# lin-shuyu/ladder-latent-data-distribution-modelling

Hardware: AMD Instinct MI355X
Metric: training images/sec (full 4-run LaDDer iteration, CelebA 128x128) (higher is better)
Workload: dtype f32; 1 GPU; BASELINE configs[2]: celeba 128x128x3 nh=512 z=64 R=2 K=30 L=100 per-GPU batch=128, 4 runs/iteration (AE step, sigma step, prior step, inner-sigma step), fitted-GM regime; global_batch=128, parallelism=dp1

## Files before the change

### include/ladder_hip.h

```cpp
#ifndef LADDER_HIP_H
#define LADDER_HIP_H

#include <stddef.h>
#include <stdint.h>

#ifdef __cplusplus
extern "C" {
#endif

typedef struct ihipStream_t* ladder_stream_t;

enum { LADDER_OK = 0, LADDER_E_SHAPE = -1, LADDER_E_ALIGN = -2, LADDER_E_WORKSPACE = -3, LADDER_E_LAUNCH = -4 };
enum { LADDER_ACT_NONE = 0, LADDER_ACT_LEAKY = 1 , LADDER_ACT_RELU = 2, LADDER_ACT_TANH = 3 };

#define LADDER_ABI_VERSION 2
int ladder_abi_version(void);
int ladder_igemm_fwd_tile(long M, int Cin, int Cout);
int ladder_conv2d_fwd_kernel_id(int N, int H, int W, int Cin, int Ho, int Wo, int Cout, int KH, int KW, int stride, int ups,
                                int pad_t, int pad_l);
int ladder_dense_fwd_nt(const float* x, const float* wT, const float* bias, float* y, int M, int K, int N, int act, ladder_stream_t stream);
int ladder_dense_bwd_data_nt(const float* dy, const float* w, float* dx, int M, int K, int N, const float* gate_y, int gate_act, ladder_stream_t stream);
int ladder_dense_fwd_is_persistent(long M, int K, int N);
int ladder_dense_bwd_weight_is_persistent(long M, int K, int N);

// ... 187 lines not shown

int ladder_conv_rgb_s2_eligible(int N, int H, int W, int Cin, int Cout, int KH, int KW, int stride, int pad_t, int pad_l);
int ladder_conv_rgb_s2_fwd(const float* x, const float* w, const float* bias, float* y, int N, int H, int W, int Cout, int act,
                           ladder_stream_t stream);
size_t ladder_conv_rgb_s2_fwd_bnstats_workspace_bytes(int N, int H, int W, int Cout);
int ladder_conv_rgb_s2_fwd_bnstats(const float* x, const float* w, const float* bias, float* y, int N, int H, int W, int Cout, int act,
                                   float* sums4 , void* ws, size_t ws_bytes,
                                   ladder_stream_t stream);
int ladder_conv_rgb_s2_fwd_f32(const float* x, const float* w, const float* bias, float* y, int N, int H, int W, int Cout, int act,
                               ladder_stream_t stream);
int ladder_conv_rgb_s2_fwd_bnstats_f32(const float* x, const float* w, const float* bias, float* y, int N, int H, int W, int Cout, int act,
                                       float* sums, void* ws, size_t ws_bytes, ladder_stream_t stream);
int ladder_conv_rgb_s2_bwd_filter_f32(const float* x, const float* dy, float* dw, float* db, int N, int H, int W, int Cout, void* ws,
                                      size_t ws_bytes, ladder_stream_t stream);
size_t ladder_conv_rgb_s2_bwd_filter_workspace_bytes(int N, int H, int W, int Cout);
int ladder_conv_rgb_s2_bwd_filter(const float* x, const float* x_absmax, const float* dy, const float* dy_absmax, float* dw, float* db,
                                  int N, int H, int W, int Cout, void* ws, size_t ws_bytes, ladder_stream_t stream);

int ladder_act_bwd(const float* dy, const float* y, float* dx, size_t n, int act, ladder_stream_t stream);

size_t ladder_bn_workspace_bytes(size_t rows, int C);
int ladder_bn_fwd_stats(const float* x, float* sums , size_t rows, int C,
                        void* ws, size_t ws_bytes, ladder_stream_t stream);
int ladder_bn_stats_from_partials(const float* partials, int nblk, float* sums , int C, ladder_stream_t stream);
int ladder_bn_fwd_stats_minmax(const float* x, float* sums4, size_t rows, int C, void* ws, size_t ws_bytes, ladder_stream_t stream);
int ladder_bn_stats_minmax_from_partials(const float* partials , int nblk, float* sums4, int C, ladder_stream_t stream);
int ladder_bn_fwd_apply_planes(const float* x, const float* sums4, double count, const float* gamma, const float* beta, float* y,
                               void* y_planes, float* mean_rstd, size_t rows, int C, float eps, int act, float* y_absmax,
                               ladder_stream_t stream);
int ladder_bn_fwd_apply(const float* x, const float* sums, double count,
                        const float* gamma, const float* beta, float* y, float* mean_rstd,
                        size_t rows, int C, float eps, int act, ladder_stream_t stream);
int ladder_bn_bwd_stats(const float* dy, const float* x, const float* mean_rstd, const float* gamma,
                        const float* beta, float* dsums , size_t rows, int C, int act,
                        void* ws, size_t ws_bytes, ladder_stream_t stream);
int ladder_bn_bwd_apply(const float* dy, const float* x, const float* mean_rstd, const float* gamma,
                        const float* beta, const float* dsums, double count, float* dx,
                        float* dgamma, float* dbeta, size_t rows, int C, int act, ladder_stream_t stream);
int ladder_bn_fwd_apply_absmax(const float* x, const float* sums, double count, const float* gamma, const float* beta, float* y,
// ... 245 lines not shown
```

### ladder_latent_data_distribution_modelling_amd/_lib.py

```python
import ctypes as C
import os

_HERE = os.path.dirname(os.path.abspath(__file__))
LIB_PATH = os.path.join(_HERE, "csrc", "libladder_hip.so")

ERRORS = {-1: "LADDER_E_SHAPE", -2: "LADDER_E_ALIGN", -3: "LADDER_E_WORKSPACE", -4: "LADDER_E_LAUNCH"}
ACT = {None: 0, "none": 0, "leaky_relu": 1, "relu": 2, "tanh": 3}

P_PIX_ABS, P_PIX_SQ, P_LOG_SDZ, P_MU2SD2_Z, P_CODE_ERR, P_CODE_SQRT, P_CODE_ABS, P_LOG_SDT, P_MU2SD2_T, P_LOGP = range(10)
P_FIXED = 16
S_NAMES = ["sigma", "mean_pixel_error", "entropy_z", "crossEntropy_prior_sg", "crossEntropy_prior",
           "l1_reconstruction_error", "l2_reconstruction_error", "reconstruction_likelihood", "sigma_regularisor",
           "elbo", "loss_ae", "inner_sigma", "mean_code_error", "code_reconstruction_likelihood",
           "code_l1_reconstruction_error", "representation_regularisor", "entropy_t",
           "crossEntropy_representation", "elbo_prior", "loss_prior",
           "_g_pix", "_g_sigma_var", "_g_code", "_g_inner_sigma_var", "_inv_B", "_inv_LB"]
S_INDEX = {n: i for i, n in enumerate(S_NAMES)}
S_COUNT = 32
ABSMAX_FLOATS = 512
ABI_VERSION = 2


class LadderElboCfg(C.Structure):
    _fields_ = [("B_global", C.c_int), ("D", C.c_int), ("Z", C.c_int), ("R", C.c_int), ("L", C.c_int),
# ... 186 lines not shown
    "ladder_dense_bwd_small": (_i, [_p, _p, _p, _p, _p, _p, _i, _i, _i, _p, _i, _p]),
    "ladder_dense_fwd_small_f32": (_i, [_p, _p, _p, _p, _i, _i, _i, _i, _p]),
    "ladder_dense_bwd_data_small_f32": (_i, [_p, _p, _p, _i, _i, _i, _p, _i, _p]),
    "ladder_dense_bwd_weight_small_f32": (_i, [_p, _p, _p, _p, _i, _i, _i, _p]),
    "ladder_dense_bwd_small_f32": (_i, [_p, _p, _p, _p, _p, _p, _i, _i, _i, _p, _i, _p]),
    "ladder_presplit_bytes": (_z, [_z, _i]),
    "ladder_presplit": (_i, [_p, _p, _p, _z, _i, _i, _p]),
    "ladder_absmax_samples": (_i, [_p, _i, _z, _p, _p]),
    "ladder_conv3x3_split_proj": (_i, [_p, _p, _p, _p, _p, _p, _p, _p] + [_i] * 8 + [_p]),
    "ladder_conv_rgb_s2_eligible": (_i, [_i] * 10),
    "ladder_conv_rgb_s2_fwd": (_i, [_p, _p, _p, _p, _i, _i, _i, _i, _i, _p]),
    "ladder_conv_rgb_s2_fwd_bnstats_workspace_bytes": (_z, [_i] * 4),
    "ladder_conv_rgb_s2_fwd_bnstats": (_i, [_p, _p, _p, _p, _i, _i, _i, _i, _i, _p, _p, _z, _p]),
    "ladder_conv_rgb_s2_fwd_f32": (_i, [_p, _p, _p, _p, _i, _i, _i, _i, _i, _p]),
    "ladder_conv_rgb_s2_fwd_bnstats_f32": (_i, [_p, _p, _p, _p, _i, _i, _i, _i, _i, _p, _p, _z, _p]),
    "ladder_bn_stats_from_partials": (_i, [_p, _i, _p, _i, _p]),
    "ladder_bn_stats_minmax_from_partials": (_i, [_p, _i, _p, _i, _p]),
    "ladder_bn_fwd_stats_minmax": (_i, [_p, _p, _z, _i, _p, _z, _p]),
    "ladder_bn_fwd_apply_planes": (_i, [_p, _p, _d, _p, _p, _p, _p, _p, _z, _i, _f, _i, _p, _p]),
    "ladder_conv_rgb_s2_bwd_filter_workspace_bytes": (_z, [_i] * 4),
    "ladder_conv_rgb_s2_bwd_filter": (_i, [_p] * 6 + [_i] * 4 + [_p, _z, _p]),
    "ladder_conv_rgb_s2_bwd_filter_f32": (_i, [_p] * 4 + [_i] * 4 + [_p, _z, _p]),
    "ladder_bn_fwd_apply_absmax": (_i, [_p, _p, _d, _p, _p, _p, _p, _z, _i, _f, _i, _p, _p]),
    "ladder_bn_bwd_apply_absmax": (_i, [_p, _p, _p, _p, _p, _p, _d, _p, _p, _p, _z, _i, _i, _p, _p]),
    "ladder_in_style_fwd_absmax": (_i, [_p, _p, _p, _p, _i, _i, _i, _f, _i, _p, _z, _p, _p]),
    "ladder_in_style_fwd_resize2x": (_i, [_p, _p, _p, _p, _i, _i, _i, _i, _f, _i, _p, _z, _p, _p]),
    "ladder_in_style_fwd_resize2x_keep": (_i, [_p, _p, _p, _p, _p, _i, _i, _i, _i, _f, _i, _p, _z, _p, _p]),
    "ladder_in_style_bwd_absmax": (_i, [_p, _p, _p, _p, _p, _p, _i, _i, _i, _i, _p, _z, _p, _p]),
    "ladder_conv1x1_smallcout_bwd_absmax": (_i, [_p, _p, _p, _p, _p, _p, C.c_long, _i, _i, _i, _p, _z, _p, C.c_long, _p]),
    "ladder_absmax": (_i, [_p, _z, _p, _p]),
    "ladder_conv3x3_wgrad_split_eligible": (_i, [_i] * 6),
# ... 78 lines not shown
```

### ladder_latent_data_distribution_modelling_amd/csrc/convrgb.hip

```cpp
#include "split16.h"
#include "igemm.h"

namespace {

constexpr int RGB_TH = 8, RGB_TW = 32, RGB_PIX = RGB_TH * RGB_TW;
constexpr int RGB_PH = 2 * RGB_TH + 1, RGB_PW = 2 * RGB_TW + 1;
constexpr int RGB_PATCH = RGB_PH * RGB_PW * 3;
constexpr int RGB_THREADS = 512;
constexpr int RGB_A_PLANE = 2 * 2 * RGB_PIX * 16;
constexpr int RGB_B_PLANE = 2 * 2 * 128 * 16;

__device__ __forceinline__ float block_max_512(float m, float* red) {
  m = wave_max(m);
  __syncthreads();
  if ((threadIdx.x & 63) == 0) red[threadIdx.x >> 6] = m;
  __syncthreads();
  float b = red[0];
#pragma unroll
  for (int w = 1; w < 8; ++w) b = fmaxf(b, red[w]);
  return b;
}

__device__ __forceinline__ float rgb_tap(const float* __restrict__ patch, int pr, int pc, int k) {
  const int tap = k / 3, ci = k - tap * 3, r = tap / 3, s = tap - r * 3;
  return patch[((2 * pr + r) * RGB_PW + 2 * pc + s) * 3 + ci];
}

constexpr int RGB_K32 = 28, RGB_LDA32 = RGB_K32 + 1;
template <bool F32>
__global__ __launch_bounds__(RGB_THREADS, 4) void conv_rgb_s2_fwd_kernel(const float* __restrict__ x, const float* __restrict__ w,
                                                                        const float* __restrict__ bias, float* __restrict__ y,
                                                                        const int N, const int H, const int W, const int Cout,
                                                                        const int act, const int tiles_n, float* __restrict__ stats_part) {
  __shared__ __attribute__((aligned(16))) unsigned char lds[2 * RGB_A_PLANE + 2 * RGB_B_PLANE];
  __shared__ __attribute__((aligned(16))) float patch[RGB_PATCH + 5];
  __shared__ float red[8];
  unsigned char* const Ab = lds;
  unsigned char* const Bb = lds + 2 * RGB_A_PLANE;

  const int tid = threadIdx.x, lane = tid & 63, wid = tid >> 6;
  const int l31 = lane & 31, lh = lane >> 5, wm = wid >> 1, wn = wid & 1;
  const int Ho = H / 2, Wo = W / 2;
  const int tile = blockIdx.x, mt = tile / tiles_n, cot = tile - mt * tiles_n, n0 = cot * 128;
  const int tw_n = Wo / RGB_TW, th_n = Ho / RGB_TH;
  const int img = mt / (tw_n * th_n), rem = mt - img * (tw_n * th_n);
  const int h0 = (rem / tw_n) * RGB_TH, w0 = (rem % tw_n) * RGB_TW;

  float xmax = 0.f;
// ... 107 lines not shown
#pragma unroll
        for (int mi = 0; mi < 2; ++mi)
#pragma unroll
          for (int ni = 0; ni < 2; ++ni) acc[mi][ni] = mfma16<true>(a[mi][pa], b[ni][sum - pa], acc[mi][ni]);
  }

  }

  const float unscale = 1.f / (cx * cw);
  float st0[2] = {0.f, 0.f}, st1[2] = {0.f, 0.f};
  float smn[2] = {INFINITY, INFINITY}, smx[2] = {-INFINITY, -INFINITY};
#pragma unroll
  for (int ni = 0; ni < 2; ++ni) {
    const int n = n0 + wn * 64 + ni * 32 + l31;
    const float bv = (bias != nullptr && n < Cout) ? bias[n] : 0.f;
#pragma unroll
    for (int mi = 0; mi < 2; ++mi) {
      float* yp = y + (((long)img * Ho + h0 + 2 * wm + mi) * Wo + w0) * Cout + n;
#pragma unroll
      for (int e = 0; e < 16; ++e) {
        const int px = (e & 3) + 8 * (e >> 2) + 4 * lh;
        const float v = ladder_act_fn(acc[mi][ni][e] * unscale + bv, act);
        if (n < Cout) yp[(long)px * Cout] = v;
        st0[ni] += v;
        st1[ni] += v * v;
        smn[ni] = fminf(smn[ni], v);
        smx[ni] = fmaxf(smx[ni], v);
      }
    }
  }
  if (stats_part != nullptr) {
    float* sred = reinterpret_cast<float*>(lds);
    __syncthreads();
#pragma unroll
    for (int ni = 0; ni < 2; ++ni) {
      const float a0 = st0[ni] + __shfl_xor(st0[ni], 32, 64), a1 = st1[ni] + __shfl_xor(st1[ni], 32, 64);
      const float a2 = fminf(smn[ni], __shfl_xor(smn[ni], 32, 64)), a3 = fmaxf(smx[ni], __shfl_xor(smx[ni], 32, 64));
      if (lh == 0) {
// ... 221 lines not shown
    __syncthreads();
  }

  float* o = part + (size_t)split * 27 * Cout;
#pragma unroll
  for (int e = 0; e < 16; ++e) {
    const int k = (e & 3) + 8 * (e >> 2) + 4 * lh;
    if (k < 27 && co_ok) o[(size_t)k * Cout + co] = acc[e];
  }
  if (bias_part != nullptr) {
    const float v = bsum + __shfl_down(bsum, 32, 64);
    if (lh == 0 && co_ok) bias_part[(size_t)split * Cout + co] = v;
  }
}

struct RgbWgradPlan { int tiles_co, splits, pps; };
RgbWgradPlan plan_rgb_wgrad(int N, int H, int W, int Cout) {
  RgbWgradPlan p;
  p.tiles_co = (Cout + 127) / 128;
  const long q_total = (long)N * (H / 2 / RW_PH) * (W / 2 / RW_PW);
  long s = (3 * 256L) / p.tiles_co;
  if (s > q_total / 4) s = q_total / 4;
  if (s < 1) s = 1;
  p.pps = (int)((q_total + s - 1) / s);
  p.splits = (int)((q_total + p.pps - 1) / p.pps);
  return p;
}

bool rgb_s2_ok(int N, int H, int W, int Cin, int Cout, int KH, int KW, int stride, int pad_t, int pad_l) {
  return N > 0 && Cin == 3 && KH == 3 && KW == 3 && stride == 2 && pad_t == 0 && pad_l == 0 && (H % 2) == 0 && (W % 2) == 0 &&
         ((H / 2) % RGB_TH) == 0 && ((W / 2) % RGB_TW) == 0 && Cout >= 32 && (Cout % 4) == 0;
}

}

extern "C" {

int ladder_conv_rgb_s2_eligible(int N, int H, int W, int Cin, int Cout, int KH, int KW, int stride, int pad_t, int pad_l) {
  return rgb_s2_ok(N, H, W, Cin, Cout, KH, KW, stride, pad_t, pad_l) ? 1 : 0;
}

static int rgb_fwd_launch(const float* x, const float* w, const float* bias, float* y, int N, int H, int W, int Cout, int act, float* stats_part,
                          ladder_stream_t stream, bool f32 = false) {
  if (!rgb_s2_ok(N, H, W, 3, Cout, 3, 3, 2, 0, 0)) return LADDER_E_SHAPE;
  if (!ladder_aligned16(y) || (bias != nullptr && !ladder_aligned16(bias))) return LADDER_E_ALIGN;
  const int tiles_n = (Cout + 127) / 128;
  const long tiles = (long)N * (H / 2 / RGB_TH) * (W / 2 / RGB_TW) * tiles_n;
  if (tiles >= (1L << 31)) return LADDER_E_SHAPE;
  if (f32)
    hipLaunchKernelGGL(conv_rgb_s2_fwd_kernel<true>, dim3((unsigned)tiles), dim3(RGB_THREADS), 0, stream, x, w, bias, y, N, H, W, Cout, act, tiles_n,
                       stats_part);
  else
    hipLaunchKernelGGL(conv_rgb_s2_fwd_kernel<false>, dim3((unsigned)tiles), dim3(RGB_THREADS), 0, stream, x, w, bias, y, N, H, W, Cout, act, tiles_n,
                       stats_part);
  LADDER_CHECK_LAUNCH();
  return LADDER_OK;
}

int ladder_conv_rgb_s2_fwd(const float* x, const float* w, const float* bias, float* y, int N, int H, int W, int Cout, int act,
                           ladder_stream_t stream) {
  return rgb_fwd_launch(x, w, bias, y, N, H, W, Cout, act, nullptr, stream);
}

size_t ladder_conv_rgb_s2_fwd_bnstats_workspace_bytes(int N, int H, int W, int Cout) {
  if (!rgb_s2_ok(N, H, W, 3, Cout, 3, 3, 2, 0, 0)) return 0;
  return (size_t)N * (H / 2 / RGB_TH) * (W / 2 / RGB_TW) * 4 * Cout * sizeof(float);
}

int ladder_conv_rgb_s2_fwd_bnstats(const float* x, const float* w, const float* bias, float* y, int N, int H, int W, int Cout, int act,
// ... 4 lines not shown
  const int rc = rgb_fwd_launch(x, w, bias, y, N, H, W, Cout, act, (float*)ws, stream);
  if (rc != LADDER_OK) return rc;
  return ladder_bn_stats_minmax_from_partials((const float*)ws, N * (H / 2 / RGB_TH) * (W / 2 / RGB_TW), sums, Cout, stream);
}

int ladder_conv_rgb_s2_fwd_f32(const float* x, const float* w, const float* bias, float* y, int N, int H, int W, int Cout, int act,
                               ladder_stream_t stream) {
  return rgb_fwd_launch(x, w, bias, y, N, H, W, Cout, act, nullptr, stream, true);
}

int ladder_conv_rgb_s2_fwd_bnstats_f32(const float* x, const float* w, const float* bias, float* y, int N, int H, int W, int Cout, int act,
                                       float* sums, void* ws, size_t ws_bytes, ladder_stream_t stream) {
  const size_t need = ladder_conv_rgb_s2_fwd_bnstats_workspace_bytes(N, H, W, Cout);
  if (need == 0 || sums == nullptr) return LADDER_E_SHAPE;
  if (ws == nullptr || ws_bytes < need) return LADDER_E_WORKSPACE;
  const int rc = rgb_fwd_launch(x, w, bias, y, N, H, W, Cout, act, (float*)ws, stream, true);
  if (rc != LADDER_OK) return rc;
  return ladder_bn_stats_minmax_from_partials((const float*)ws, N * (H / 2 / RGB_TH) * (W / 2 / RGB_TW), sums, Cout, stream);
}

int ladder_conv_rgb_s2_bwd_filter_f32(const float* x, const float* dy, float* dw, float* db, int N, int H, int W, int Cout, void* ws,
                                      size_t ws_bytes, ladder_stream_t stream) {
  if (!rgb_s2_ok(N, H, W, 3, Cout, 3, 3, 2, 0, 0)) return LADDER_E_SHAPE;
  if (!ladder_aligned16(dw)) return LADDER_E_ALIGN;
  const RgbWgradPlan p = plan_rgb_wgrad(N, H, W, Cout);
  if (ws == nullptr || ws_bytes < (size_t)p.splits * (27 * (size_t)Cout + Cout) * sizeof(float)) return LADDER_E_WORKSPACE;
  const WgradTail t = wgrad_tail(ws, p.splits, (size_t)27 * Cout, Cout, dw, db);
  hipLaunchKernelGGL(conv_rgb_s2_wgrad_f32_kernel, dim3(p.tiles_co * p.splits), dim3(RW_THREADS), 0, stream, x, dy, t.part, t.bias_part, N, H, W, Cout,
                     p.tiles_co, p.pps);
  return t.reduce(stream);
}

size_t ladder_conv_rgb_s2_bwd_filter_workspace_bytes(int N, int H, int W, int Cout) {
  if (!rgb_s2_ok(N, H, W, 3, Cout, 3, 3, 2, 0, 0)) return 0;
  const RgbWgradPlan p = plan_rgb_wgrad(N, H, W, Cout);
  return (size_t)p.splits * (27 * (size_t)Cout + Cout) * sizeof(float);
}

int ladder_conv_rgb_s2_bwd_filter(const float* x, const float* x_absmax, const float* dy, const float* dy_absmax, float* dw, float* db, int N,
                                  int H, int W, int Cout, void* ws, size_t ws_bytes, ladder_stream_t stream) {
  if (!rgb_s2_ok(N, H, W, 3, Cout, 3, 3, 2, 0, 0) || x_absmax == nullptr || dy_absmax == nullptr) return LADDER_E_SHAPE;
  if (!ladder_aligned16(dy) || !ladder_aligned16(dw)) return LADDER_E_ALIGN;
  if (ws == nullptr || ws_bytes < ladder_conv_rgb_s2_bwd_filter_workspace_bytes(N, H, W, Cout)) return LADDER_E_WORKSPACE;
  const RgbWgradPlan p = plan_rgb_wgrad(N, H, W, Cout);
  const WgradTail t = wgrad_tail(ws, p.splits, (size_t)27 * Cout, Cout, dw, db);
  hipLaunchKernelGGL(conv_rgb_s2_wgrad_kernel, dim3(p.tiles_co * p.splits), dim3(RW_THREADS), 0, stream, x, dy, t.part, t.bias_part, N, H, W, Cout,
                     p.tiles_co, p.pps, x_absmax, dy_absmax);
// ... 5 lines not shown
```

### ladder_latent_data_distribution_modelling_amd/csrc/norm.hip

```cpp
#include "split16.h"
#include "norm_util.h"

namespace {

template <bool MINMAX>
struct MomentsRow {
  using Sum = double;
  static constexpr bool kMinMax = MINMAX;
  const float* x;
  double* ws;
  float* wsmm;
  template <int V> struct Coef {};
  template <int V> using In = Lanes<float, V>;
  template <int V> struct Acc {
    Lanes<double, V> s0 = lanes_fill<double, V>(0.0), s1 = lanes_fill<double, V>(0.0);
    Lanes<float, V> mn = lanes_fill<float, V>(INFINITY), mx = lanes_fill<float, V>(-INFINITY);
  };
  template <int V> __device__ __forceinline__ Coef<V> coef(int, int) const { return {}; }
  template <int V> __device__ __forceinline__ In<V> load(size_t i) const { return lanes_load<V>(x + i); }
  template <int V> __device__ __forceinline__ void add(Acc<V>& a, const In<V>& v, const Coef<V>&) const {
#pragma unroll
    for (int j = 0; j < V; ++j) {
      const double d = (double)v.v[j];
      a.s0.v[j] += d;
// ... 863 lines not shown

int ladder_bn_bwd_stats(const float* dy, const float* x, const float* mean_rstd, const float* gamma, const float* beta,
                        float* dsums, size_t rows, int C, int act, void* ws, size_t ws_bytes, ladder_stream_t stream) {
  if (rows == 0 || C <= 0) return LADDER_E_SHAPE;
  const size_t nblk = stats_nblk(rows);
  if (ws_bytes < nblk * 2 * (size_t)C * sizeof(float)) return LADDER_E_WORKSPACE;
  const BnBwdRow row = {dy, x, mean_rstd, gamma, beta, (float*)ws, act};
  if (vec4_ok(C, x, dy)) stage1_launch<4>(row, rows, C, nblk, stream);
  else stage1_launch<1>(row, rows, C, nblk, stream);
  hipLaunchKernelGGL((colstats_stage2<64, 16, 1, false, float, float>), dim3((2 * C + 63) / 64), dim3(1024), 0, stream, (const float*)ws, 2,
                     (const float*)nullptr, 0, 0, dsums, (int)nblk, C);
  LADDER_CHECK_LAUNCH();
  return LADDER_OK;
}

int ladder_bn_bwd_apply(const float* dy, const float* x, const float* mean_rstd, const float* gamma, const float* beta,
                        const float* dsums, double count, float* dx, float* dgamma, float* dbeta, size_t rows, int C, int act,
                        ladder_stream_t stream) {
  return ladder_bn_bwd_apply_absmax(dy, x, mean_rstd, gamma, beta, dsums, count, dx, dgamma, dbeta, rows, C, act, nullptr, stream);
}

int ladder_bn_bwd_apply_absmax(const float* dy, const float* x, const float* mean_rstd, const float* gamma, const float* beta,
                               const float* dsums, double count, float* dx, float* dgamma, float* dbeta, size_t rows, int C, int act,
                               float* dx_absmax, ladder_stream_t stream) {
  if (rows == 0 || C <= 0 || count <= 0) return LADDER_E_SHAPE;
  const size_t n = rows * (size_t)C;
  const bool v4 = dx != nullptr && vec4_ok(C, x, dy, dx);
  if (dx_absmax != nullptr && !v4) return LADDER_E_SHAPE;
  const bool pgrad = dgamma != nullptr && dbeta != nullptr;
  static const bool fold = getenv("LADDER_DISABLE_BN_FOLD") == nullptr;
// ... 191 lines not shown
```

### ladder_latent_data_distribution_modelling_amd/engine.py

```python
import os

import numpy as np
import torch

from . import _lib as L
from . import arch
from . import layers as _layers
from .comm import Comm, VirtualComm, VirtualGroup, run_virtual_ranks, _NoComm, _DoneWork, _TracedWork
from .layers import (ADAM_B1, ADAM_B2, ADAM_EPS, BN_EPS, DEFAULT_PRECISION, IN_EPS, PRECISION_NOTES, PRECISIONS, BatchNormAct, Conv2D, Ctx, Dense,
                     DepthToSpace, InstanceNormStyleAct, ParamStore, PlanesOnly, Resize, _p, _timed, add_, pad_symmetric, plan_decoder)
from .mixture import DeviceMixture
from .mixture_forms import check_status_word, family, sized_workspace
from .profiler import KernelProfiler


def set_profiler(prof):
    _layers.PROF = prof


class Encoder:
    def __init__(self, ctx, ps, cfg):
        self.ctx, self.cfg = ctx, cfg
        self.exp = cfg["exp_name"]
        self.convs, self.bns = [], []
        for i, (cin, cout, k, s, pad, act, bn) in enumerate(arch.encoder_convs(cfg)):
            self.convs.append(Conv2D(ctx, ps, "encoder/" + arch.tfname("conv2d", i), k, cin, cout, s, pad, act, bias_grad=not bn, want_bn_sums=bool(bn)))
            self.bns.append(BatchNormAct(ctx, ps, "encoder/" + arch.tfname("batch_normalization", i), cout, "leaky_relu") if bn else None)
        feat, hid = arch.encoder_flat_dim(cfg), arch.encoder_hidden(cfg)
        self.hidden = Dense(ctx, ps, "encoder/dense", feat, hid, "leaky_relu") if hid is not None else None
        feat = hid if hid is not None else feat
        Z = int(cfg["code_size"])
        self.head_mu = Dense(ctx, ps, "encoder/code_mean", feat, Z, None)
        self.head_sd = Dense(ctx, ps, "encoder/code_std_dev", feat, Z, "relu")

    def forward(self, x):
        h = pad_symmetric(self.ctx, x, 2) if self.exp != "celeba" else x
        for i, (conv, bn) in enumerate(zip(self.convs, self.bns)):
            h = conv.forward(h)
            if bn is not None:
                nxt = self.convs[i + 1] if i + 1 < len(self.convs) else None
                h = bn.forward(h, sums=conv.bn_sums, planes=nxt.planes_demand(h.shape) if nxt is not None else (False, True))
            conv.bn_sums = None
        self.conv_shape = h.shape
        h = h.reshape(h.shape[0], -1)
        if self.hidden is not None:
            h = self.hidden.forward(h)
        return self.head_mu.forward(h), self.head_sd.forward(h)

    def backward(self, dmu, dsd_raw, wgrad=True, need_input_dx=False):
        dh = self.head_mu.backward(dmu, wgrad=wgrad)
        add_(self.ctx, dh, self.head_sd.backward(dsd_raw, wgrad=wgrad, act_done=True))
        if self.hidden is not None:
            dh = self.hidden.backward(dh, wgrad=wgrad)
        dh = dh.reshape(self.conv_shape)
        for i in range(len(self.convs) - 1, -1, -1):
            if self.bns[i] is not None:
                dh = self.bns[i].backward(dh, wgrad=wgrad)
            dh = self.convs[i].backward(dh, need_dx=(i > 0 or need_input_dx), wgrad=wgrad)
        if need_input_dx and self.exp != "celeba":
            N, Hp, Wp, C = dh.shape
            dx = self.ctx.empty(N, Hp - 4, Wp - 4, C)
            L.call("ladder_pad_symmetric_bwd", _p(dh), _p(dx), N, Hp - 4, Wp - 4, C, 2, self.ctx.stream)
            dh = dx
        return dh if need_input_dx else None


class MnistDecoder:
    def __init__(self, ctx, ps, cfg):
        self.ctx = ctx
        width, r0, convs = arch.mnist_decoder_convs(cfg)
        self.dense = Dense(ctx, ps, "decoder/dense", int(cfg["code_size"]), width, "leaky_relu")
        self.d2s0 = DepthToSpace(ctx, r0)
        self.convs, self.d2s = [], []
# ... 197 lines not shown

class LadderEngine:

    def __init__(self, cfg, device="cuda:0", values=None, seed=1, comm=None, noise_seed=1234):
        self.cfg = cfg
        if comm is None and bool(int(cfg.get("deterministic_allreduce", 0))):
            comm = Comm(deterministic=True)
        self.ctx = Ctx(device, comm)
        prec = str(cfg.get("matmul_precision", DEFAULT_PRECISION))
        if prec not in PRECISIONS:
            raise ValueError("matmul_precision %r: expected one of %s" % (prec, sorted(PRECISIONS)))
        self.ctx.ns = PRECISIONS[prec]
        self.ctx.up2 = int(cfg.get("upsample_fused_convs", 4 if prec == "f32" else 2))
        self.ctx.fuse_fwd = int(cfg.get("fused_projected_forward", 2))
        self.ctx.fuse_bwd_proj = int(cfg.get("fused_projection_backward", 1))
        self.precision = prec
        if self.ctx.comm.rank == 0:
            print("Contraction precision (config key matmul_precision): {} -- {}".format(prec, PRECISION_NOTES[prec]))
        self.ps = ParamStore(cfg, self.ctx, values, seed)
        self.encoder = Encoder(self.ctx, self.ps, cfg)
        self.decoder = (CelebADecoder if cfg["exp_name"] == "celeba" else MnistDecoder)(self.ctx, self.ps, cfg)
        self.has_inner = cfg["prior"] in ("ours", "hierarchical")
        self.hier = cfg["prior"] == "hierarchical"
        self.gmm_z = cfg["prior"] == "GMM"
        self.vamp = cfg["prior"] == "vampPrior"
        if cfg["prior"] not in ("ours", "hierarchical", "GMM", "vampPrior", "standard_gaussian"):
            raise ValueError("unknown prior %r" % cfg["prior"])
        if self.vamp:
            self.encoder_p = Encoder(self.ctx.local(), self.ps, cfg)
            self._enc_range = self.ps.prefix_range("ae", "encoder/")
        self.inner = InnerVAE(self.ctx, self.ps, cfg) if self.has_inner else None
        self.Z = int(cfg["code_size"])
        self.R = int(cfg["code_size"]) if cfg["prior"] in ("GMM", "vampPrior") else int(cfg.get("representation_size", 1))
        self.K = int(cfg.get("n_mixtures", 1))
        self.Lmc = int(cfg.get("n_MC_samples", 1))
        self.D = int(cfg["dim_input_x"]) * int(cfg["dim_input_y"]) * int(cfg["dim_input_channel"])
        self.lvp = float(cfg["latent_variance_precision"])
        self.partials = self.ctx.zeros(L.P_FIXED + self.Z + self.R)
        self.scalars = self.ctx.zeros(L.S_COUNT)
        self.noise_seed = int(noise_seed) + 7919 * self.ctx.comm.rank
        self.rng_counter = torch.zeros(1, dtype=torch.int64, device=self.ctx.device)
        self._run_calls = 0
        self.mixture = None
        self.use_graphs = False
# ... 554 lines not shown
```

### ladder_latent_data_distribution_modelling_amd/layers.py

```python
import functools
import os
from collections import namedtuple

import numpy as np
import torch

from . import _lib as L
from . import arch
from .comm import Comm, _NoComm

BN_EPS = 1e-3
IN_EPS = 1e-6
ADAM_B1, ADAM_B2, ADAM_EPS = 0.9, 0.95, 1e-8


def _p(t):
    return None if t is None else t.data_ptr()


PRECISIONS = {"f32": 0, "bf16x3": 2, "bf16x6": 3, "f16x3": 4}
DEFAULT_PRECISION = "f32"

PRECISION_NOTES = {
    "f32": "native fp32 MFMA (v_mfma_f32_32x32x2_f32), bit-exact fp32 FMA chains",
# ... 1013 lines not shown
        ctx.comm.allreduce_(dsums, "C2 bwd " + self.name.split("/")[-1])
        dx = torch.empty_like(x) if need_dx else None
        dx_amax = ctx.new_amax() if (need_dx and ctx.ns == 4 and C % 4 == 0) else None
        L.call("ladder_bn_bwd_apply_absmax", _p(dy), _p(x), _p(self.mean_rstd), _p(gam), _p(bet), _p(dsums), self.count, _p(dx),
               _p(self.ps.g[self.name + "/gamma"]) if wgrad else None, _p(self.ps.g[self.name + "/beta"]) if wgrad else None,
               rows, C, L.ACT[self.act], _p(dx_amax), ctx.stream)
        if dx is not None:
            ctx.set_amax(dx, dx_amax)
        if wgrad and ctx.comm.world > 1:
            for t in (self.ps.g[self.name + "/gamma"], self.ps.g[self.name + "/beta"]):
                L.call("ladder_axpy", _p(t), _p(t), t.numel(), 1.0 / ctx.comm.world, 0, ctx.stream)
        self.x = None
        return dx


class InstanceNormStyleAct:

    def __init__(self, ctx, C, act):
        self.ctx, self.C, self.act = ctx, C, act

    def forward(self, x, style):
        N, H, W, C = x.shape
        y = torch.empty_like(x)
        self.mean_rstd = self.ctx.empty(N, 2 * C)
        wsp, wsn = self.ctx.ws(L.query("ladder_in_style_workspace_bytes", N, H * W, C))
        y_amax = self.ctx.new_amax() if (self.ctx.ns == 4 and C % 4 == 0) else None
        L.call("ladder_in_style_fwd_absmax", _p(x), _p(style), _p(y), _p(self.mean_rstd), N, H * W, C, IN_EPS, L.ACT[self.act],
               wsp, wsn, _p(y_amax), self.ctx.stream)
        self.ctx.set_amax(y, y_amax)
        self.x, self.style = x, style
# ... 97 lines not shown
```

Baseline: 7208 images/sec.

## Fuse first encoder conv with batchnorm via recompute in forward and backward

Measured after the change: 7279 images/sec, median of 6. No clear change (+1.0%).

```diff
diff --git a/include/ladder_hip.h b/include/ladder_hip.h
--- a/include/ladder_hip.h
+++ b/include/ladder_hip.h
@@ -225,6 +225,15 @@
 int ladder_conv_rgb_s2_bwd_filter_f32(const float* x, const float* dy, float* dw, float* db, int N, int H, int W, int Cout, void* ws,
                                       size_t ws_bytes, ladder_stream_t stream);
 size_t ladder_conv_rgb_s2_bwd_filter_workspace_bytes(int N, int H, int W, int Cout);
+int ladder_conv_rgb_s2_bn_apply_f32(const float* x, const float* w, const float* bias, const float* sums, double count, const float* gamma,
+                                    const float* beta, float* y, float* mean_rstd, int N, int H, int W, int Cout, int act, float eps, int bn_act,
+                                    ladder_stream_t stream);
+int ladder_conv_rgb_s2_bn_bwd_stats_f32(const float* x, const float* w, const float* bias, const float* dy, const float* mean_rstd, const float* gamma,
+                                        const float* beta, float* dsums, int N, int H, int W, int Cout, int bn_act, void* ws, size_t ws_bytes,
+                                        ladder_stream_t stream);
+int ladder_conv_rgb_s2_bn_bwd_filter_f32(const float* x, const float* w, const float* bias, const float* dy, const float* mean_rstd, const float* gamma,
+                                         const float* beta, const float* dsums, double count, float* dw, float* dgamma, float* dbeta, int N, int H,
+                                         int W, int Cout, int bn_act, void* ws, size_t ws_bytes, ladder_stream_t stream);
 int ladder_conv_rgb_s2_bwd_filter(const float* x, const float* x_absmax, const float* dy, const float* dy_absmax, float* dw, float* db,
                                   int N, int H, int W, int Cout, void* ws, size_t ws_bytes, ladder_stream_t stream);
 
@@ -234,6 +243,7 @@
 int ladder_bn_fwd_stats(const float* x, float* sums , size_t rows, int C,
                         void* ws, size_t ws_bytes, ladder_stream_t stream);
 int ladder_bn_stats_from_partials(const float* partials, int nblk, float* sums , int C, ladder_stream_t stream);
+int ladder_bn_bwd_stats_from_partials(const float* partials, int nblk, float* dsums, int C, ladder_stream_t stream);
 int ladder_bn_fwd_stats_minmax(const float* x, float* sums4, size_t rows, int C, void* ws, size_t ws_bytes, ladder_stream_t stream);
 int ladder_bn_stats_minmax_from_partials(const float* partials , int nblk, float* sums4, int C, ladder_stream_t stream);
 int ladder_bn_fwd_apply_planes(const float* x, const float* sums4, double count, const float* gamma, const float* beta, float* y,
diff --git a/ladder_latent_data_distribution_modelling_amd/_lib.py b/ladder_latent_data_distribution_modelling_amd/_lib.py
--- a/ladder_latent_data_distribution_modelling_amd/_lib.py
+++ b/ladder_latent_data_distribution_modelling_amd/_lib.py
@@ -224,7 +224,11 @@
     "ladder_conv_rgb_s2_fwd_bnstats": (_i, [_p, _p, _p, _p, _i, _i, _i, _i, _i, _p, _p, _z, _p]),
     "ladder_conv_rgb_s2_fwd_f32": (_i, [_p, _p, _p, _p, _i, _i, _i, _i, _i, _p]),
     "ladder_conv_rgb_s2_fwd_bnstats_f32": (_i, [_p, _p, _p, _p, _i, _i, _i, _i, _i, _p, _p, _z, _p]),
+    "ladder_conv_rgb_s2_bn_apply_f32": (_i, [_p, _p, _p, _p, _d, _p, _p, _p, _p, _i, _i, _i, _i, _i, _f, _i, _p]),
+    "ladder_conv_rgb_s2_bn_bwd_stats_f32": (_i, [_p] * 8 + [_i] * 5 + [_p, _z, _p]),
+    "ladder_conv_rgb_s2_bn_bwd_filter_f32": (_i, [_p] * 8 + [_d] + [_p] * 3 + [_i] * 5 + [_p, _z, _p]),
     "ladder_bn_stats_from_partials": (_i, [_p, _i, _p, _i, _p]),
+    "ladder_bn_bwd_stats_from_partials": (_i, [_p, _i, _p, _i, _p]),
     "ladder_bn_stats_minmax_from_partials": (_i, [_p, _i, _p, _i, _p]),
     "ladder_bn_fwd_stats_minmax": (_i, [_p, _p, _z, _i, _p, _z, _p]),
     "ladder_bn_fwd_apply_planes": (_i, [_p, _p, _d, _p, _p, _p, _p, _p, _z, _i, _f, _i, _p, _p]),
diff --git a/ladder_latent_data_distribution_modelling_amd/csrc/convrgb.hip b/ladder_latent_data_distribution_modelling_amd/csrc/convrgb.hip
--- a/ladder_latent_data_distribution_modelling_amd/csrc/convrgb.hip
+++ b/ladder_latent_data_distribution_modelling_amd/csrc/convrgb.hip
@@ -1,5 +1,6 @@
 #include "split16.h"
 #include "igemm.h"
+#include "norm_util.h"
 
 namespace {
 
@@ -27,11 +28,20 @@
 }
 
 constexpr int RGB_K32 = 28, RGB_LDA32 = RGB_K32 + 1;
-template <bool F32>
+enum { RGB_STORE = 0, RGB_STATS = 1, RGB_BN = 2 };
+struct RgbBn {
+  const float *sums, *gamma, *beta;
+  float* mean_rstd;
+  double count;
+  float eps;
+  int act;
+};
+template <bool F32, int MODE = RGB_STORE>
 __global__ __launch_bounds__(RGB_THREADS, 4) void conv_rgb_s2_fwd_kernel(const float* __restrict__ x, const float* __restrict__ w,
                                                                         const float* __restrict__ bias, float* __restrict__ y,
                                                                         const int N, const int H, const int W, const int Cout,
-                                                                        const int act, const int tiles_n, float* __restrict__ stats_part) {
+                                                                        const int act, const int tiles_n, float* __restrict__ stats_part,
+                                                                        const RgbBn bn = RgbBn{}) {
   __shared__ __attribute__((aligned(16))) unsigned char lds[2 * RGB_A_PLANE + 2 * RGB_B_PLANE];
   __shared__ __attribute__((aligned(16))) float patch[RGB_PATCH + 5];
   __shared__ float red[8];
@@ -169,6 +179,18 @@
   for (int ni = 0; ni < 2; ++ni) {
     const int n = n0 + wn * 64 + ni * 32 + l31;
     const float bv = (bias != nullptr && n < Cout) ? bias[n] : 0.f;
+    NormCoef<1> kc = {{0.f}, {0.f}, {0.f}, {0.f}};
+    if constexpr (MODE == RGB_BN) {
+      if (n < Cout) {
+        bn_moments(bn.sums, Cout, n, bn.count, bn.eps, kc.mean[0], kc.rstd[0]);
+        kc.scale[0] = bn.gamma[n];
+        kc.shift[0] = bn.beta[n];
+        if (mt == 0 && wm == 0 && lh == 0) {
+          bn.mean_rstd[n] = kc.mean[0];
+          bn.mean_rstd[Cout + n] = kc.rstd[0];
+        }
+      }
+    }
 #pragma unroll
     for (int mi = 0; mi < 2; ++mi) {
       float* yp = y + (((long)img * Ho + h0 + 2 * wm + mi) * Wo + w0) * Cout + n;
@@ -176,7 +198,12 @@
       for (int e = 0; e < 16; ++e) {
         const int px = (e & 3) + 8 * (e >> 2) + 4 * lh;
         const float v = ladder_act_fn(acc[mi][ni][e] * unscale + bv, act);
-        if (n < Cout) yp[(long)px * Cout] = v;
+        if constexpr (MODE == RGB_BN) {
+          if (n < Cout) yp[(long)px * Cout] = norm_act(v, kc, bn.act);
+          continue;
+        }
+        if constexpr (MODE == RGB_STORE)
+          if (n < Cout) yp[(long)px * Cout] = v;
         st0[ni] += v;
         st1[ni] += v * v;
         smn[ni] = fminf(smn[ni], v);
@@ -428,6 +455,146 @@
   }
 }
 
+template <bool APPLY>
+__global__ __launch_bounds__(RW_THREADS, APPLY ? 3 : 4) void conv_rgb_s2_bn_bwd_kernel(
+    const float* __restrict__ x, const float* __restrict__ w, const float* __restrict__ bias, const float* __restrict__ dy,
+    const float* __restrict__ mean_rstd, const float* __restrict__ gamma, const float* __restrict__ beta, const float* __restrict__ dsums,
+    const float inv_count, float* __restrict__ part, float* __restrict__ dgamma, float* __restrict__ dbeta, const int N, const int H, const int W,
+    const int Cout, const int tiles_co, const int patches_per_split, const int bn_act) {
+  __shared__ float A32[RW_PIX * RW_LDA32];
+  __shared__ float patch[RW_PATCH + 1];
+  const int tid = threadIdx.x, lane = tid & 63, wv = tid >> 6;
+  const int l31 = lane & 31, lh = lane >> 5;
+  const int split = blockIdx.x / tiles_co, co0 = (blockIdx.x - split * tiles_co) * 128;
+  const int Ho = H / 2, Wo = W / 2, WP = Wo / RW_PW, HP = Ho / RW_PH;
+  const int q_total = N * HP * WP;
+  const int q0 = split * patches_per_split, q1 = min(q_total, q0 + patches_per_split);
+  const int co = co0 + wv * 32 + l31;
+  const bool co_ok = co < Cout;
+
+  float wf[RGB_K32 / 2];
+#pragma unroll
+  for (int ks = 0; ks < RGB_K32 / 2; ++ks) {
+    const int k = 2 * ks + lh;
+    wf[ks] = (k < 27 && co_ok) ? w[(long)k * Cout + co] : 0.f;
+  }
+  const float bv = (bias != nullptr && co_ok) ? bias[co] : 0.f;
+  NormCoef<1> kc = {{0.f}, {0.f}, {0.f}, {0.f}};
+  float m1 = 0.f, m2 = 0.f;
+  if (co_ok) {
+    kc = bn_coef<1>(mean_rstd, gamma, beta, Cout, co);
+    if constexpr (APPLY) {
+      m1 = dsums[co] * inv_count;
+      m2 = dsums[Cout + co] * inv_count;
+    }
+  }
+  if constexpr (APPLY) {
+    if (dgamma != nullptr && blockIdx.x == 0)
+      for (int c = tid; c < Cout; c += RW_THREADS) {
+        dbeta[c] = dsums[c];
+        dgamma[c] = dsums[Cout + c];
+      }
+  }
+
+  f32x16 acc;
+#pragma unroll
+  for (int e = 0; e < 16; ++e) acc[e] = 0.f;
+  Lanes<float, 1> s0 = {{0.f}}, s1 = {{0.f}};
+  float xr[RW_XU];
+  auto decode = [&](int q, int& img, int& h0, int& w0) {
+    img = q / (HP * WP);
+    const int rem = q - img * (HP * WP), hp = rem / WP;
+    h0 = hp * RW_PH;
+    w0 = (rem - hp * WP) * RW_PW;
+  };
+  auto load_x = [&](int q) {
+    int img, h0, w0;
+    decode(q, img, h0, w0);
+#pragma unroll
+    for (int i = 0; i < RW_XU; ++i) {
+      const int v = tid + i * RW_THREADS;
+      const int r = v / (RW_XW * 3), c3 = v - r * (RW_XW * 3);
+      const int hi = 2 * h0 + r, wi3 = 2 * w0 * 3 + c3;
+      xr[i] = (v < RW_PATCH && hi < H && wi3 < W * 3) ? x[((long)img * H + hi) * W * 3 + wi3] : 0.f;
+    }
+  };
+
+  if (q0 < q1) load_x(q0);
+  for (int q = q0; q < q1; ++q) {
+    float b[RW_PIX / 2];
+    {
+      int img, h0, w0;
+      decode(q, img, h0, w0);
+      const float* du = dy + (((long)img * Ho + h0) * Wo + w0) * Cout;
+      const unsigned loff = (unsigned)(co + 4 * lh * Cout);
+#pragma unroll
+      for (int i = 0; i < RW_PIX / 2; ++i) {
+        const int mi = i >> 4, e = i & 15;
+        const float* pk = du + ((long)mi * Wo + (e & 3) + 8 * (e >> 2)) * Cout;
+        b[i] = co_ok ? pk[loff] : 0.f;
+      }
+    }
+#pragma unroll
+    for (int i = 0; i < RW_XU; ++i)
+      if (tid + i * RW_THREADS < RW_PATCH) patch[tid + i * RW_THREADS] = xr[i];
+    __syncthreads();
+    if (q + 1 < q1) load_x(q + 1);
+    {
+      const int p = tid & (RW_PIX - 1), kq = tid >> 6, pr = p >> 5, pc = p & 31;
+#pragma unroll
+      for (int j = 0; j < 8; ++j) {
+        const int k = kq * 8 + j;
+        const int tap = k / 3, ci = k - tap * 3, r = tap / 3, sx = tap - r * 3;
+        A32[p * RW_LDA32 + k] = k < 27 ? patch[((2 * pr + r) * RW_XW + 2 * pc + sx) * 3 + ci] : 0.f;
+      }
+    }
+    __syncthreads();
+#pragma unroll
+    for (int mi = 0; mi < RW_PH; ++mi) {
+      f32x16 c;
+#pragma unroll
+      for (int e = 0; e < 16; ++e) c[e] = 0.f;
+      const float* Afr = A32 + (mi * 32 + l31) * RW_LDA32 + lh;
+#pragma unroll
+      for (int ks = 0; ks < RGB_K32 / 2; ++ks) c = __builtin_amdgcn_mfma_f32_32x32x2f32(Afr[2 * ks], wf[ks], c, 0, 0, 0);
+#pragma unroll
+      for (int e = 0; e < 16; ++e) {
+        const Lanes<float, 1> cv = {{c[e] + bv}}, dv = {{b[16 * mi + e]}};
+        if constexpr (APPLY) {
+          Lanes<float, 1> xh, grad;
+          norm_bwd_terms<1>(cv, kc, bn_act, xh, grad);
+          b[16 * mi + e] = norm_dx<1>(xh, dv, grad, kc, {{m1}}, {{m2}}).v[0];
+        } else {
+          norm_bwd_accumulate<1>(cv, dv, kc, bn_act, s0, s1);
+        }
+      }
+      if constexpr (APPLY) {
+#pragma unroll
+        for (int e = 0; e < 16; ++e) {
+          const float a = A32[(mi * 32 + (e & 3) + 8 * (e >> 2) + 4 * lh) * RW_LDA32 + l31];
+          acc = __builtin_amdgcn_mfma_f32_32x32x2f32(a, b[16 * mi + e], acc, 0, 0, 0);
+        }
+      }
+    }
+    __syncthreads();
+  }
+
+  if constexpr (APPLY) {
+    float* o = part + (size_t)split * 27 * Cout;
+#pragma unroll
+    for (int e = 0; e < 16; ++e) {
+      const int k = (e & 3) + 8 * (e >> 2) + 4 * lh;
+      if (k < 27 && co_ok) o[(size_t)k * Cout + co] = acc[e];
+    }
+  } else {
+    const float t0 = s0.v[0] + __shfl_xor(s0.v[0], 32, 64), t1 = s1.v[0] + __shfl_xor(s1.v[0], 32, 64);
+    if (lh == 0 && co_ok) {
+      part[((size_t)split * 2 + 0) * Cout + co] = t0;
+      part[((size_t)split * 2 + 1) * Cout + co] = t1;
+    }
+  }
+}
+
 struct RgbWgradPlan { int tiles_co, splits, pps; };
 RgbWgradPlan plan_rgb_wgrad(int N, int H, int W, int Cout) {
   RgbWgradPlan p;
@@ -455,18 +622,26 @@
 }
 
 static int rgb_fwd_launch(const float* x, const float* w, const float* bias, float* y, int N, int H, int W, int Cout, int act, float* stats_part,
-                          ladder_stream_t stream, bool f32 = false) {
+                          ladder_stream_t stream, bool f32 = false, int mode = RGB_STORE, const RgbBn& bn = RgbBn{}) {
   if (!rgb_s2_ok(N, H, W, 3, Cout, 3, 3, 2, 0, 0)) return LADDER_E_SHAPE;
   if (!ladder_aligned16(y) || (bias != nullptr && !ladder_aligned16(bias))) return LADDER_E_ALIGN;
   const int tiles_n = (Cout + 127) / 128;
   const long tiles = (long)N * (H / 2 / RGB_TH) * (W / 2 / RGB_TW) * tiles_n;
   if (tiles >= (1L << 31)) return LADDER_E_SHAPE;
-  if (f32)
-    hipLaunchKernelGGL(conv_rgb_s2_fwd_kernel<true>, dim3((unsigned)tiles), dim3(RGB_THREADS), 0, stream, x, w, bias, y, N, H, W, Cout, act, tiles_n,
-                       stats_part);
+  if (f32 && mode == RGB_STATS)
+    hipLaunchKernelGGL((conv_rgb_s2_fwd_kernel<true, RGB_STATS>), dim3((unsigned)tiles), dim3(RGB_THREADS), 0, stream, x, w, bias, y, N, H, W, Cout, act,
+                       tiles_n, stats_part, bn);
+  else if (f32 && mode == RGB_BN)
+    hipLaunchKernelGGL((conv_rgb_s2_fwd_kernel<true, RGB_BN>), dim3((unsigned)tiles), dim3(RGB_THREADS), 0, stream, x, w, bias, y, N, H, W, Cout, act,
+                       tiles_n, stats_part, bn);
+  else if (mode != RGB_STORE)
+    return LADDER_E_SHAPE;
+  else if (f32)
+    hipLaunchKernelGGL((conv_rgb_s2_fwd_kernel<true>), dim3((unsigned)tiles), dim3(RGB_THREADS), 0, stream, x, w, bias, y, N, H, W, Cout, act, tiles_n,
+                       stats_part, bn);
   else
-    hipLaunchKernelGGL(conv_rgb_s2_fwd_kernel<false>, dim3((unsigned)tiles), dim3(RGB_THREADS), 0, stream, x, w, bias, y, N, H, W, Cout, act, tiles_n,
-                       stats_part);
+    hipLaunchKernelGGL((conv_rgb_s2_fwd_kernel<false>), dim3((unsigned)tiles), dim3(RGB_THREADS), 0, stream, x, w, bias, y, N, H, W, Cout, act, tiles_n,
+                       stats_part, bn);
   LADDER_CHECK_LAUNCH();
   return LADDER_OK;
 }
@@ -501,9 +676,18 @@
   const size_t need = ladder_conv_rgb_s2_fwd_bnstats_workspace_bytes(N, H, W, Cout);
   if (need == 0 || sums == nullptr) return LADDER_E_SHAPE;
   if (ws == nullptr || ws_bytes < need) return LADDER_E_WORKSPACE;
-  const int rc = rgb_fwd_launch(x, w, bias, y, N, H, W, Cout, act, (float*)ws, stream, true);
+  const int rc = rgb_fwd_launch(x, w, bias, y, N, H, W, Cout, act, (float*)ws, stream, true, y == nullptr ? RGB_STATS : RGB_STORE);
   if (rc != LADDER_OK) return rc;
   return ladder_bn_stats_minmax_from_partials((const float*)ws, N * (H / 2 / RGB_TH) * (W / 2 / RGB_TW), sums, Cout, stream);
+}
+
+int ladder_conv_rgb_s2_bn_apply_f32(const float* x, const float* w, const float* bias, const float* sums, double count, const float* gamma,
+                                    const float* beta, float* y, float* mean_rstd, int N, int H, int W, int Cout, int act, float eps, int bn_act,
+                                    ladder_stream_t stream) {
+  if (sums == nullptr || gamma == nullptr || beta == nullptr || y == nullptr || mean_rstd == nullptr || count <= 0) return LADDER_E_SHAPE;
+  if ((reinterpret_cast<uintptr_t>(sums) & 7u) != 0) return LADDER_E_ALIGN;
+  const RgbBn bn = {sums, gamma, beta, mean_rstd, count, eps, bn_act};
+  return rgb_fwd_launch(x, w, bias, y, N, H, W, Cout, act, nullptr, stream, true, RGB_BN, bn);
 }
 
 int ladder_conv_rgb_s2_bwd_filter_f32(const float* x, const float* dy, float* dw, float* db, int N, int H, int W, int Cout, void* ws,
@@ -518,6 +702,33 @@
   return t.reduce(stream);
 }
 
+int ladder_conv_rgb_s2_bn_bwd_stats_f32(const float* x, const float* w, const float* bias, const float* dy, const float* mean_rstd, const float* gamma,
+                                        const float* beta, float* dsums, int N, int H, int W, int Cout, int bn_act, void* ws, size_t ws_bytes,
+                                        ladder_stream_t stream) {
+  if (!rgb_s2_ok(N, H, W, 3, Cout, 3, 3, 2, 0, 0) || dsums == nullptr || mean_rstd == nullptr || gamma == nullptr || beta == nullptr) return LADDER_E_SHAPE;
+  const RgbWgradPlan p = plan_rgb_wgrad(N, H, W, Cout);
+  if (ws == nullptr || ws_bytes < (size_t)p.splits * 2 * Cout * sizeof(float)) return LADDER_E_WORKSPACE;
+  hipLaunchKernelGGL(conv_rgb_s2_bn_bwd_kernel<false>, dim3(p.tiles_co * p.splits), dim3(RW_THREADS), 0, stream, x, w, bias, dy, mean_rstd, gamma, beta,
+                     (const float*)nullptr, 0.f, (float*)ws, (float*)nullptr, (float*)nullptr, N, H, W, Cout, p.tiles_co, p.pps, bn_act);
+  LADDER_CHECK_LAUNCH();
+  return ladder_bn_bwd_stats_from_partials((const float*)ws, p.splits, dsums, Cout, stream);
+}
+
+int ladder_conv_rgb_s2_bn_bwd_filter_f32(const float* x, const float* w, const float* bias, const float* dy, const float* mean_rstd, const float* gamma,
+                                         const float* beta, const float* dsums, double count, float* dw, float* dgamma, float* dbeta, int N, int H,
+                                         int W, int Cout, int bn_act, void* ws, size_t ws_bytes, ladder_stream_t stream) {
+  if (!rgb_s2_ok(N, H, W, 3, Cout, 3, 3, 2, 0, 0) || dsums == nullptr || mean_rstd == nullptr || gamma == nullptr || beta == nullptr || dw == nullptr ||
+      count <= 0 || (dgamma == nullptr) != (dbeta == nullptr))
+    return LADDER_E_SHAPE;
+  if (!ladder_aligned16(dw)) return LADDER_E_ALIGN;
+  const RgbWgradPlan p = plan_rgb_wgrad(N, H, W, Cout);
+  if (ws == nullptr || ws_bytes < (size_t)p.splits * 27 * Cout * sizeof(float)) return LADDER_E_WORKSPACE;
+  const WgradTail t = wgrad_tail(ws, p.splits, (size_t)27 * Cout, Cout, dw, nullptr);
+  hipLaunchKernelGGL(conv_rgb_s2_bn_bwd_kernel<true>, dim3(p.tiles_co * p.splits), dim3(RW_THREADS), 0, stream, x, w, bias, dy, mean_rstd, gamma, beta,
+                     dsums, (float)(1.0 / count), t.part, dgamma, dbeta, N, H, W, Cout, p.tiles_co, p.pps, bn_act);
+  return t.reduce(stream);
+}
+
 size_t ladder_conv_rgb_s2_bwd_filter_workspace_bytes(int N, int H, int W, int Cout) {
   if (!rgb_s2_ok(N, H, W, 3, Cout, 3, 3, 2, 0, 0)) return 0;
   const RgbWgradPlan p = plan_rgb_wgrad(N, H, W, Cout);
diff --git a/ladder_latent_data_distribution_modelling_amd/csrc/norm.hip b/ladder_latent_data_distribution_modelling_amd/csrc/norm.hip
--- a/ladder_latent_data_distribution_modelling_amd/csrc/norm.hip
+++ b/ladder_latent_data_distribution_modelling_amd/csrc/norm.hip
@@ -901,6 +901,14 @@
   return LADDER_OK;
 }
 
+int ladder_bn_bwd_stats_from_partials(const float* partials, int nblk, float* dsums, int C, ladder_stream_t stream) {
+  if (nblk <= 0 || C <= 0 || partials == nullptr || dsums == nullptr) return LADDER_E_SHAPE;
+  hipLaunchKernelGGL((colstats_stage2<64, 16, 1, false, float, float>), dim3((2 * C + 63) / 64), dim3(1024), 0, stream, partials, 2,
+                     (const float*)nullptr, 0, 0, dsums, nblk, C);
+  LADDER_CHECK_LAUNCH();
+  return LADDER_OK;
+}
+
 int ladder_bn_bwd_apply(const float* dy, const float* x, const float* mean_rstd, const float* gamma, const float* beta,
                         const float* dsums, double count, float* dx, float* dgamma, float* dbeta, size_t rows, int C, int act,
                         ladder_stream_t stream) {
diff --git a/ladder_latent_data_distribution_modelling_amd/engine.py b/ladder_latent_data_distribution_modelling_amd/engine.py
--- a/ladder_latent_data_distribution_modelling_amd/engine.py
+++ b/ladder_latent_data_distribution_modelling_amd/engine.py
@@ -8,7 +8,7 @@
 from . import layers as _layers
 from .comm import Comm, VirtualComm, VirtualGroup, run_virtual_ranks, _NoComm, _DoneWork, _TracedWork
 from .layers import (ADAM_B1, ADAM_B2, ADAM_EPS, BN_EPS, DEFAULT_PRECISION, IN_EPS, PRECISION_NOTES, PRECISIONS, BatchNormAct, Conv2D, Ctx, Dense,
-                     DepthToSpace, InstanceNormStyleAct, ParamStore, PlanesOnly, Resize, _p, _timed, add_, pad_symmetric, plan_decoder)
+                     DepthToSpace, FirstLayerPair, InstanceNormStyleAct, ParamStore, PlanesOnly, Resize, _p, _timed, add_, pad_symmetric, plan_decoder)
 from .mixture import DeviceMixture
 from .mixture_forms import check_status_word, family, sized_workspace
 from .profiler import KernelProfiler
@@ -19,13 +19,14 @@
 
 
 class Encoder:
-    def __init__(self, ctx, ps, cfg):
+    def __init__(self, ctx, ps, cfg, input_grad=False):
         self.ctx, self.cfg = ctx, cfg
         self.exp = cfg["exp_name"]
         self.convs, self.bns = [], []
         for i, (cin, cout, k, s, pad, act, bn) in enumerate(arch.encoder_convs(cfg)):
             self.convs.append(Conv2D(ctx, ps, "encoder/" + arch.tfname("conv2d", i), k, cin, cout, s, pad, act, bias_grad=not bn, want_bn_sums=bool(bn)))
             self.bns.append(BatchNormAct(ctx, ps, "encoder/" + arch.tfname("batch_normalization", i), cout, "leaky_relu") if bn else None)
+        self.first = FirstLayerPair(ctx, self.convs[0], self.bns[0], input_grad)
         feat, hid = arch.encoder_flat_dim(cfg), arch.encoder_hidden(cfg)
         self.hidden = Dense(ctx, ps, "encoder/dense", feat, hid, "leaky_relu") if hid is not None else None
         feat = hid if hid is not None else feat
@@ -36,9 +37,13 @@
     def forward(self, x):
         h = pad_symmetric(self.ctx, x, 2) if self.exp != "celeba" else x
         for i, (conv, bn) in enumerate(zip(self.convs, self.bns)):
+            nxt = self.convs[i + 1] if i + 1 < len(self.convs) else None
+            if i == 0:
+                r = conv.route(h.shape)
+                h = self.first.forward(h, planes=nxt.planes_demand((r.N, r.Ho, r.Wo, conv.cout)) if (bn is not None and nxt is not None) else (False, True))
+                continue
             h = conv.forward(h)
             if bn is not None:
-                nxt = self.convs[i + 1] if i + 1 < len(self.convs) else None
                 h = bn.forward(h, sums=conv.bn_sums, planes=nxt.planes_demand(h.shape) if nxt is not None else (False, True))
             conv.bn_sums = None
         self.conv_shape = h.shape
@@ -53,10 +58,11 @@
         if self.hidden is not None:
             dh = self.hidden.backward(dh, wgrad=wgrad)
         dh = dh.reshape(self.conv_shape)
-        for i in range(len(self.convs) - 1, -1, -1):
+        for i in range(len(self.convs) - 1, 0, -1):
             if self.bns[i] is not None:
                 dh = self.bns[i].backward(dh, wgrad=wgrad)
-            dh = self.convs[i].backward(dh, need_dx=(i > 0 or need_input_dx), wgrad=wgrad)
+            dh = self.convs[i].backward(dh, need_dx=True, wgrad=wgrad)
+        dh = self.first.backward(dh, wgrad=wgrad, need_input_dx=need_input_dx)
         if need_input_dx and self.exp != "celeba":
             N, Hp, Wp, C = dh.shape
             dx = self.ctx.empty(N, Hp - 4, Wp - 4, C)
@@ -284,6 +290,7 @@
         self.ctx.up2 = int(cfg.get("upsample_fused_convs", 4 if prec == "f32" else 2))
         self.ctx.fuse_fwd = int(cfg.get("fused_projected_forward", 2))
         self.ctx.fuse_bwd_proj = int(cfg.get("fused_projection_backward", 1))
+        self.ctx.first_layer_recompute = int(cfg.get("first_layer_recompute", 1))
         self.precision = prec
         if self.ctx.comm.rank == 0:
             print("Contraction precision (config key matmul_precision): {} -- {}".format(prec, PRECISION_NOTES[prec]))
@@ -297,7 +304,7 @@
         if cfg["prior"] not in ("ours", "hierarchical", "GMM", "vampPrior", "standard_gaussian"):
             raise ValueError("unknown prior %r" % cfg["prior"])
         if self.vamp:
-            self.encoder_p = Encoder(self.ctx.local(), self.ps, cfg)
+            self.encoder_p = Encoder(self.ctx.local(), self.ps, cfg, input_grad=True)
             self._enc_range = self.ps.prefix_range("ae", "encoder/")
         self.inner = InnerVAE(self.ctx, self.ps, cfg) if self.has_inner else None
         self.Z = int(cfg["code_size"])
diff --git a/ladder_latent_data_distribution_modelling_amd/layers.py b/ladder_latent_data_distribution_modelling_amd/layers.py
--- a/ladder_latent_data_distribution_modelling_amd/layers.py
+++ b/ladder_latent_data_distribution_modelling_amd/layers.py
@@ -1051,6 +1051,81 @@
         return dx
 
 
+FirstLayerPlan = namedtuple("FirstLayerPlan", "pair route")
+
+
+class FirstLayerPair:
+
+    def __init__(self, ctx, conv, bn, input_grad=False):
+        self.ctx, self.conv, self.bn, self.input_grad = ctx, conv, bn, bool(input_grad)
+        self._plans, self.plan = {}, None
+
+    def plan_for(self, shape):
+        ctx, conv = self.ctx, self.conv
+        r = conv.route(shape)
+        key = (tuple(shape[:3]), ctx.ns, int(getattr(ctx, "first_layer_recompute", 1)), r.fwd.fn, r.wgrad.fn)
+        if key not in self._plans:
+            pair = bool(key[2] and not self.input_grad and ctx.ns == 0 and self.bn is not None and r.stats
+                        and r.fwd.fn == "ladder_conv_rgb_s2_fwd_bnstats_f32" and r.wgrad.fn == "ladder_conv_rgb_s2_bwd_filter_f32")
+            self._plans[key] = FirstLayerPlan(pair, r)
+        return self._plans[key]
+
+    def _operands(self):
+        bn = self.bn
+        return self.conv._wb(), (_p(bn.ps.w[bn.name + "/gamma"]), _p(bn.ps.w[bn.name + "/beta"]))
+
+    def forward(self, x, planes=(False, True)):
+        ctx, conv, bn = self.ctx, self.conv, self.bn
+        plan = self.plan = self.plan_for(x.shape)
+        if not plan.pair:
+            h = conv.forward(x)
+            if bn is not None:
+                h = bn.forward(h, sums=conv.bn_sums, planes=planes)
+            conv.bn_sums = None
+            return h
+        r, C = plan.route, conv.cout
+        (w, b), (gam, bet) = self._operands()
+        sums = ctx.empty(6 * C)
+        wsp, wsn = ctx.ws(r.fwd.ws)
+        L.call(r.fwd.fn, _p(x), w, b, None, r.N, r.H, r.W, C, L.ACT[conv.act], _p(sums), wsp, wsn, ctx.stream)
+        ctx.comm.allreduce_(sums[:4 * C].view(torch.float64), "C2 fwd " + bn.name.split("/")[-1])
+        bn.count = float(r.N * r.Ho * r.Wo) * ctx.comm.world
+        bn.mean_rstd, bn.x = ctx.empty(2 * C), None
+        y = ctx.empty(r.N, r.Ho, r.Wo, C)
+        L.call("ladder_conv_rgb_s2_bn_apply_f32", _p(x), w, b, _p(sums), bn.count, gam, bet, _p(y), _p(bn.mean_rstd), r.N, r.H, r.W, C,
+               L.ACT[conv.act], BN_EPS, L.ACT[bn.act], ctx.stream)
+        conv._keep("pair", x, None, r)
+        return y
+
+    def backward(self, dy, wgrad=True, need_input_dx=False):
+        ctx, conv, bn, plan = self.ctx, self.conv, self.bn, self.plan
+        if plan is None or not plan.pair:
+            if bn is not None:
+                dy = bn.backward(dy, wgrad=wgrad)
+            return conv.backward(dy, need_dx=need_input_dx, wgrad=wgrad)
+        try:
+            if need_input_dx:
+                raise RuntimeError("%s: the recompute form of the first layer has no backward-data (construct the pair with input_grad=True)" % conv.name)
+            if not wgrad:
+                return None
+            r, x, C = plan.route, conv.kept.x, conv.cout
+            (w, b), (gam, bet) = self._operands()
+            dsums = ctx.empty(2 * C)
+            wsp, wsn = ctx.ws(r.wgrad.ws)
+            L.call("ladder_conv_rgb_s2_bn_bwd_stats_f32", _p(x), w, b, _p(dy), _p(bn.mean_rstd), gam, bet, _p(dsums), r.N, r.H, r.W, C, L.ACT[bn.act],
+                   wsp, wsn, ctx.stream)
+            ctx.comm.allreduce_(dsums, "C2 bwd " + bn.name.split("/")[-1])
+            gg, gb = bn.ps.g[bn.name + "/gamma"], bn.ps.g[bn.name + "/beta"]
+            L.call("ladder_conv_rgb_s2_bn_bwd_filter_f32", _p(x), w, b, _p(dy), _p(bn.mean_rstd), gam, bet, _p(dsums), bn.count, conv._grads()[0], _p(gg),
+                   _p(gb), r.N, r.H, r.W, C, L.ACT[bn.act], wsp, wsn, ctx.stream)
+            if ctx.comm.world > 1:
+                for t in (gg, gb):
+                    L.call("ladder_axpy", _p(t), _p(t), t.numel(), 1.0 / ctx.comm.world, 0, ctx.stream)
+            return None
+        finally:
+            conv.kept = None
+
+
 class InstanceNormStyleAct:
 
     def __init__(self, ctx, C, act):
```
